# slatedb/slatedb

Measured on AMD Instinct MI355X. Metric: GiB/s device-resident SST block encode+bloom, 64 MiB sorted KV, 1/2/4/8 GPU, higher is better.
Workload: dtype u8

## Files before the change

slatedb_amd/csrc/sdb_api.cpp:

```cpp
#include <hip/hip_runtime.h>
#include <stdint.h>

#include <algorithm>
#include <mutex>
#include <vector>

#include "../../include/slatedb_amd.h"
#include "sdb_decode.h"
#include "sdb_bloom.h"
#include "sdb_compact.h"
#include "sdb_reads.h"

using namespace sdb;

namespace {

inline hipStream_t S(void *s) { return reinterpret_cast<hipStream_t>(s); }

uint16_t num_probes_for(uint32_t bpk) { return (uint16_t)((float)bpk * 0.69f); }

uint64_t filter_bytes_for(uint64_t n, uint32_t bpk) {
    uint32_t bits = (uint32_t)n * bpk;
    return bits / 8u + (bits % 8u != 0);
}
// ... 127 lines not shown
    s.nfacts = (uint32_t)((n + kFactsEntries - 1) / kFactsEntries);
    encode_ws_layout(n, s.wso);
    {
        uint32_t g = 16;
        while ((uint64_t)g * g < s.nchunks) g++;
        s.group = g;
    }
    *standalone_bloom = false;
    if (want_filter && prefix_filter(p)) {
        s.prefix_bloom = 1;
        s.bloom_len = 0;
        *standalone_bloom = true;
    } else if (want_filter && n) {
        const BloomPlan pl = bloom_plan(n, s.num_probes, fb, kChunk);
        if (bloom_plan_fits(pl)) {
            s.bloom_fused = 1;
            s.bpl = pl;
            s.slot_cap = bloom_slot_cap(pl);
        } else {
            *standalone_bloom = true;
        }
    }
    return s;
}

SstSet set_header(const sdb_sst_params *p) {
    SstSet P{};
    P.block_size = p->block_size;
    P.restart_interval = p->sst_version == 2 ? p->restart_interval : 1;
    P.version = p->sst_version;
    P.wal = p->sst_type == SDB_SST_WAL;
    const uint64_t look = (uint64_t)p->block_size / 12 + 2;
    P.seg_look = (uint32_t)(look < kSegLook ? look : kSegLook);
    return P;
}
}

extern "C" {

uint64_t sdb_encode_workspace_bytes(uint64_t n, const sdb_sst_params *params) {
    if (!params) return 0;
    return sst_ws_bytes(n, params) + 256;
}

uint64_t sdb_encode_ssts_workspace_bytes(uint32_t count, const sdb_kv_batch *batches, const sdb_sst_params *params) {
    if (!params || (count && !batches)) return 0;
    uint64_t t = 256;
    for (uint32_t i = 0; i < count; i++) t += sst_ws_bytes(batches[i].n, params);
    return t;
}

sdb_status sdb_encode_ssts(uint32_t count, const sdb_kv_batch *batches, const sdb_sst_params *p,
                           const sdb_sst_out *outs, void *workspace, uint64_t workspace_bytes, void *stream) {
    sdb_status st = check_params(p);
    if (st) return st;
    if (count && (!batches || !outs)) return SDB_INVALID_ARGUMENT;
    for (uint32_t i = 0; i < count; i++)
        if ((st = check_sst(&batches[i], p, &outs[i]))) return st;
    if (!device_ok()) return SDB_DEVICE_ERROR;
    if (!workspace || workspace_bytes < sdb_encode_ssts_workspace_bytes(count, batches, p)) return SDB_INVALID_ARGUMENT;
    hipStream_t s = S(stream);
    uint8_t *ws = ws_align(workspace);
    SstSet P = set_header(p);
    size_t bin_lds = 0, fill_lds = 0;
    auto flush = [&]() -> bool {
        const bool ok = launch_encode_set(P, bin_lds, fill_lds, s) == hipSuccess;
// ... 602 lines not shown
```

slatedb_amd/csrc/sdb_compact.hip:

```cpp
#include <hip/hip_runtime.h>

#include "sdb_compact.h"
#include "sdb_device.h"

namespace sdb {

namespace {

constexpr uint32_t kPfxThreads = 256;

SDB_DEV uint32_t run_of(const MergeArgs &a, uint64_t g) {
    uint32_t r = 0;
    for (uint32_t k = 1; k < a.nruns; k++) r += g >= a.r[k].base ? 1u : 0u;
    return r;
}

SDB_DEV RunDesc run_desc(const MergeArgs &a, uint32_t run) {
    RunDesc d = a.r[0];
    for (uint32_t k = 1; k < a.nruns; k++) {
        const RunDesc &c = a.r[k];
        const bool m = run == k;
        d.n = m ? c.n : d.n;
        d.base = m ? c.base : d.base;
        d.key_arena = m ? c.key_arena : d.key_arena;
// ... 728 lines not shown
                    e = n;
                    break;
                }
                acc += s_bb[o];
                if (acc > max_sst) {
                    if (j + 1 < n) cut[++ns] = j + 1;
                    acc = 0;
                    e = j + 1;
                    entry_pt = (e % kChunk) == 0;
                    continue;
                }
                entry_pt = j / kChunk != k;
                e = j;
            }
            s_stage = want;
        }
        __syncthreads();
        const uint64_t sv = s_stage;
        const uint64_t want = (uint64_t)(uint32_t)__builtin_amdgcn_readfirstlane((int)(uint32_t)sv) |
                              ((uint64_t)(uint32_t)__builtin_amdgcn_readfirstlane((int)(uint32_t)(sv >> 32)) << 32);
        if (want == kCutDone) break;
        if (want & kCutTables) {
            const uint64_t g = want & ~kCutTables, k0 = g * G, nk = k0 + G < K ? G : K - k0;
            for (uint32_t x = tid; x < nk * W; x += kCutThreads) {
                const uint32_t q = x / W, o = x - q * W;
                const uint64_t kk = k0 + q, ccs = kk * kChunk, cce = ccs + kChunk < n ? ccs + kChunk : n;
                s_cx[x] = ccs + o < cce ? a.tab_exit[kk * L + o] : 0xFFFFFFFFu;
                s_cb[x] = ccs + o < cce ? a.tab_bytes[kk * L + o] : 0;
            }
            gstaged = g;
        } else {
            const uint64_t cs = want * kChunk, ce = cs + kChunk < n ? cs + kChunk : n;
            for (uint64_t x = cs + tid; x < ce; x += kCutThreads) {
                s_next[x - cs] = a.next[x];
                s_bb[x - cs] = a.bbytes[x];
            }
            staged = want;
        }
        __syncthreads();
    }
    if (tid == 0) {
        if (n) cut[++ns] = n;
        *num = ns;
    }
}

__global__ void k_cut_offsets(const uint64_t *cut, const uint64_t *num, const uint64_t *key_off, const uint64_t *val_off,
                              uint64_t *out) {
    const uint64_t ns = *num;
    for (uint64_t i = (uint64_t)blockIdx.x * blockDim.x + threadIdx.x; i <= ns; i += (uint64_t)gridDim.x * blockDim.x) {
        const uint64_t c = cut[i];
        out[2 * i] = key_off[c];
        out[2 * i + 1] = val_off[c];
    }
}

__global__ void k_cx_blocks(CxInputs in, uint64_t *start, uint64_t *end) {
    const uint64_t nb = in.nblocks;
    for (uint64_t k = (uint64_t)blockIdx.x * blockDim.x + threadIdx.x; k < nb; k += (uint64_t)gridDim.x * blockDim.x) {
        uint32_t lo = 0, hi = in.n - 1;
        while (lo < hi) {
            const uint32_t mid = (lo + hi + 1) >> 1;
            if (in.first_block[mid] <= k) lo = mid;
            else hi = mid - 1;
        }
        const uint64_t j = k - in.first_block[lo], d = (uint64_t)(uintptr_t)in.data[lo] - in.base;
        start[k] = d + in.block_off[lo][j];
        end[k] = d + in.block_off[lo][j + 1];
// ... 156 lines not shown
```

slatedb_amd/csrc/sdb_encode.h:

```cpp
#pragma once
#include <hip/hip_runtime.h>
#include <stdint.h>

#include "../../include/slatedb_amd.h"
#include "sdb_workspace.h"

namespace sdb {

constexpr uint32_t kChunk = 2048;
constexpr uint32_t kResolveLds = 96 * 1024;
#ifndef SDB_EMIT_CRC_MFMA
#define SDB_EMIT_CRC_SLICE
#endif
#ifdef SDB_EMIT_CRC_SLICE
constexpr uint32_t kCrcLds = 36 * 1024;
#else
constexpr uint32_t kCrcLds = 56 * 1024;
#endif
constexpr uint32_t kImgCap = 4096 + 64;
constexpr uint32_t kStageCap = 4096;
constexpr uint32_t kStageGuard = 64;
constexpr uint32_t kKeyStageCap = 1024;
constexpr uint32_t kPieceRowMax = 4000, kPieceKeyMax = 960, kPieceValMax = 3968;
constexpr uint32_t kSegLook = 1024;
// ... 23 lines not shown
};
struct BloomSlots {
    uint32_t *count;
    uint32_t *slot;
    uint32_t cap;
};

struct BlockDesc {
    uint32_t s, e;
    uint64_t off;
    uint64_t vs, ve, ks, ke;
    uint32_t bb, route;
};
enum : uint32_t { kRouteImage = 0, kRouteWorkgroup = 1, kRoutePieces = 2 };
enum : uint32_t { kChunkHuge = 1, kChunkCarry = 2 };

struct EncodeArgs {
    const uint8_t *key_bytes;
    const uint64_t *key_off;
    const uint8_t *val_bytes;
    const uint64_t *val_off;
    const uint8_t *kind;
    const uint64_t *seq;
    const int64_t *create_ts;
    const int64_t *expire_ts;
    const uint8_t *ts_mask;
    uint64_t n;
    uint32_t block_size;
    uint32_t restart_interval;
    uint32_t version;
    uint32_t wal;
    uint32_t nchunks;
    uint32_t seg_look;
    uint32_t *lcp;
    uint32_t *szr, *sznr;
    uint32_t nfacts;
    uint32_t *row_scratch;
    uint32_t *next;
    uint32_t *bbytes;
    uint32_t *tab_exit;
    uint32_t *tab_cnt;
    uint64_t *tab_bytes;
    uint32_t *anchor_e;
    uint32_t *anchor_blk;
    uint64_t *anchor_byte;
    unsigned long long *err;
    uint32_t *wmax;
    uint32_t *slow_count;
    uint32_t *slow_list;
    uint32_t *big_count;
    uint32_t *big_list;
    BlockDesc *desc;
    uint64_t *stat_part;
    uint32_t *huge_part;
    uint32_t *wmax_part;
    unsigned long long *err_part;
    uint32_t *gtab_exit;
    uint32_t *gtab_cnt;
    uint64_t *gtab_bytes;
    uint32_t *pre_exit;
    uint32_t *pre_cnt;
    uint64_t *pre_bytes;
    uint32_t *anchor_arrived;
    uint32_t *mode;
    uint32_t group;
    uint32_t bloom_fused;
    BloomPlan bpl;
    BloomSlots bq;
    uint8_t *bloom_out;
    uint32_t *done;
    uint32_t nprep_wg;
    uint32_t seg_lds;
    uint8_t *out_data;
    uint64_t *out_block_off;
    uint32_t *out_block_first;
    uint32_t *out_index_key_len;
    uint16_t *out_block_stats;
    uint64_t data_cap, block_cap;
    sdb_sst_summary *summary;
    uint64_t bloom_len;
    uint32_t num_probes, filter_built;
    const uint64_t *bloom_len_dev;
};

#define SDB_ENCODE_WS(X)                                                                                      \
    X(lcp, uint32_t, n + 1)                                                                                   \
    X(szr, uint32_t, n + 1)                                                                                   \
    X(sznr, uint32_t, n + 1)                                                                                  \
    X(row_scratch, uint32_t, n + 1)                                                                           \
    X(next, uint32_t, n + 1)                                                                                  \
    X(bbytes, uint32_t, n + 1)                                                                                \
    X(tab_exit, uint32_t, nt)                                                                                 \
    X(tab_cnt, uint32_t, nt)                                                                                  \
    X(tab_bytes, uint64_t, nt)                                                                                \
    X(anchor_e, uint32_t, nc + 2)                                                                             \
    X(anchor_blk, uint32_t, nc + 2)                                                                           \
    X(anchor_byte, uint64_t, nc + 2)                                                                          \
    X(err, unsigned long long, 1)                                                                             \
    X(wmax, uint32_t, 1)                                                                                      \
    X(slow_count, uint32_t, 1)                                                                                \
    X(slow_list, uint32_t, n + 1)                                                                             \
    X(big_count, uint32_t, 1)                                                                                 \
    X(big_list, uint32_t, n + 1)                                                                              \
    X(desc, BlockDesc, n + 1)                                                                                 \
    X(stat_part, uint64_t, 5 * (nf + 1))                                                                      \
    X(huge_part, uint32_t, nf + 1)                                                                            \
    X(wmax_part, uint32_t, nc + 1)                                                                            \
    X(err_part, unsigned long long, nf + 1)                                                                   \
    X(done, uint32_t, 2)                                                                                      \
    X(gtab_exit, uint32_t, nt)                                                                                \
    X(gtab_cnt, uint32_t, nt)                                                                                 \
    X(gtab_bytes, uint64_t, nt)                                                                               \
    X(pre_exit, uint32_t, nt)                                                                                 \
    X(pre_cnt, uint32_t, nt)                                                                                  \
    X(pre_bytes, uint64_t, nt)                                                                                \
    X(anchor_arrived, uint32_t, 1)                                                                            \
    X(mode, uint32_t, 1)                                                                                      \
    X(bloom_len_dev, const uint64_t, 1)
enum WsField {
#define X(name, T, count) kWs_##name,
    SDB_ENCODE_WS(X)
#undef X
    kWsTail,
    kWsFields
// ... 26 lines not shown
                              const int32_t *qlens, uint64_t n, uint8_t *result, hipStream_t st);

constexpr uint32_t kMaxSsts = 8;
struct SstSlot {
    const uint8_t *key_bytes;
    const uint64_t *key_off;
    const uint8_t *val_bytes;
    const uint64_t *val_off;
    const uint8_t *kind;
    const uint64_t *seq;
    const int64_t *create_ts;
    const int64_t *expire_ts;
    const uint8_t *ts_mask;
    uint64_t n;
    uint8_t *out_data;
    uint64_t *out_block_off;
    uint32_t *out_block_first;
    uint32_t *out_index_key_len;
    uint16_t *out_block_stats;
    uint64_t data_cap, block_cap;
    sdb_sst_summary *summary;
    uint8_t *bloom_out;
    uint64_t bloom_len;
    uint8_t *ws;
    uint32_t num_probes, filter_built, bloom_fused;
    uint32_t prefix_bloom;
    uint32_t nchunks, nfacts, group, slot_cap;
    BloomPlan bpl;
    uint32_t wso[kWsFields];
};
struct SstSet {
    uint32_t count;
    uint32_t block_size, restart_interval, version, wal, seg_look;
    uint32_t max_facts, max_chunks, max_groups, max_tiles, max_slices, pad;
    SstSlot s[kMaxSsts];
};

__host__ __device__ inline EncodeArgs make_args(const SstSet &P, uint32_t i) {
    const SstSlot &s = P.s[i];
    EncodeArgs a{};
    a.key_bytes = s.key_bytes;
    a.key_off = s.key_off;
    a.val_bytes = s.val_bytes;
    a.val_off = s.val_off;
    a.kind = s.kind;
    a.seq = s.seq;
    a.create_ts = s.create_ts;
    a.expire_ts = s.expire_ts;
    a.ts_mask = s.ts_mask;
    a.n = s.n;
    a.block_size = P.block_size;
    a.restart_interval = P.restart_interval;
    a.version = P.version;
    a.wal = P.wal;
    a.nchunks = s.nchunks;
    a.seg_look = P.seg_look;
    a.nfacts = s.nfacts;
#define X(name, T, count) a.name = (T *)(s.ws + ((uint64_t)s.wso[kWs_##name] << 8));
    SDB_ENCODE_WS(X)
#undef X
    if (!s.prefix_bloom) a.bloom_len_dev = nullptr;
    a.group = s.group;
    a.bloom_fused = s.bloom_fused;
    a.bpl = s.bpl;
    a.bq.cap = s.slot_cap;
    bloom_slots_bind(a.bq, s.bpl, s.ws + ((uint64_t)s.wso[kWsTail] << 8));
    a.bloom_out = s.bloom_out;
    a.nprep_wg = s.nchunks;
    a.seg_lds = kSegLds;
    a.out_data = s.out_data;
    a.out_block_off = s.out_block_off;
    a.out_block_first = s.out_block_first;
    a.out_index_key_len = s.out_index_key_len;
    a.out_block_stats = s.out_block_stats;
    a.data_cap = s.data_cap;
    a.block_cap = s.block_cap;
    a.summary = s.summary;
    a.bloom_len = s.bloom_len;
    a.num_probes = s.num_probes;
    a.filter_built = s.filter_built;
    return a;
}

hipError_t launch_encode_set(const SstSet &P, size_t bin_lds, size_t fill_lds, hipStream_t st);
hipError_t launch_encode_empty(EncodeArgs a, hipStream_t st);
hipError_t launch_encode_prep(const SstSet &P, hipStream_t st);

enum Stage { kStBloom = 0, kStFacts, kStSeg, kStAnchor, kStBlocks, kStEmit, kStEmitBig, kStBloomFill, kNumStages };
void stage_mark(hipStream_t st, int stage, bool begin);
bool stage_timing_on();

BloomPlan bloom_plan(uint64_t n, uint32_t k, uint64_t bitmap_bytes, uint32_t tile_keys = 0);
uint64_t bloom_workspace_bytes(uint64_t n, uint32_t k, uint64_t bitmap_bytes);
hipError_t launch_bloom_build(const uint8_t *key_bytes, const uint64_t *key_off, uint64_t n,
                              uint32_t num_probes, uint8_t *bitmap, uint64_t bitmap_bytes, uint8_t *w,
                              hipStream_t st);
hipError_t launch_bloom_query(const uint8_t *bitmap, uint64_t bitmap_bytes, uint32_t num_probes,
                              const uint8_t *key_bytes, const uint64_t *key_off, uint64_t n,
                              uint8_t *result, hipStream_t st);

}
static_assert(sdb::kSegSpan % sdb::kSegThreads == 0 && sdb::kChunk % 64 == 0, "k_seg geometry");
static_assert(sdb::kEmitLds <= 160 * 1024, "k_emit LDS");
static_assert(sizeof(sdb::SstSet) <= 4096, "SstSet is passed as kernel arguments");
```

slatedb_amd/csrc/sdb_encode.hip:

```cpp
#include <stdlib.h>

#include <atomic>
#include <mutex>

#include "sdb_bloom.h"
#include "sdb_crc.h"
#include "sdb_crc_mfma.h"

namespace sdb {

#ifndef SDB_SEG_WAVES
#define SDB_SEG_WAVES 8
#endif
#ifdef SDB_PHASE_TIMING
__device__ uint64_t g_phase[1024][8];
#define PHASE_MARK(i)                                                              \
    do {                                                                           \
        __syncthreads();                                                           \
        if (threadIdx.x == 0 && blockIdx.x < 1024) g_phase[blockIdx.x][i] = __builtin_amdgcn_s_memtime(); \
    } while (0)
__device__ uint64_t g_wave_phase[8192][8];
__device__ uint64_t g_wave_rt[8192][4];
#define WAVE_T(var)                                     \
    uint64_t var = __builtin_amdgcn_s_memtime();        \
// ... 75 lines not shown
        else if (x1) lcp = 8 + (__builtin_ctzll(x1) >> 3);
        else if (nmin <= 16) lcp = nmin;
        else lcp = 16 + lcp_bytes(a.key_bytes + in.pko + 16, nmin - 16, a.key_bytes + in.ko0 + 16, nmin - 16);
        if (klen == 0) err = SDB_EMPTY_KEY;
        else if (!a.wal && plen > 0 && lcp == klen && klen < plen) err = SDB_INVALID_ARGUMENT;
    }
    if (!err && klen == 0) err = SDB_EMPTY_KEY;
    const uint32_t ts8 = 8u * (((m & SDB_TS_CREATE) != 0) + ((m & SDB_TS_EXPIRE) != 0));
    if (a.version == 2) {
        if (!err && (klen > 0xFFFFFFFFull || vlen > 0xFFFFFFFFull)) err = SDB_LIMIT_EXCEEDED;
        uint32_t kl = (uint32_t)klen, vl = (uint32_t)vlen, suf = kl - lcp;
        f.s_nr = varint_len(lcp) + varint_len(suf) + varint_len(vl) + suf + vl + 9 + ts8;
        f.s_r = 1 + varint_len(kl) + varint_len(vl) + kl + vl + 9 + ts8;
    } else {
        if (!err && (klen > 0xFFFF || vlen > 0xFFFFFFFFull)) err = SDB_LIMIT_EXCEEDED;
        f.s_r = (uint32_t)(4 + klen + 9 + ts8 + (kd == SDB_KIND_TOMBSTONE ? 0 : 4 + vlen));
        f.s_nr = f.s_r;
    }
    f.lcp = lcp;
    f.klen = klen;
    f.vlen = vlen;
    f.kind = kd;
    f.err = err;
    return f;
}

SDB_DEV EntryFacts entry_facts(const EncodeArgs &a, uint64_t i) {
    FactsIn in;
    facts_load_offsets(a, i, in);
    facts_load_keys(a, in);
    return facts_finish(a, i, in);
}

template <int CTRL>
SDB_DEV uint64_t dpp_or_own(uint64_t own, uint64_t v) {
    const uint32_t lo = (uint32_t)__builtin_amdgcn_update_dpp((int)(uint32_t)own, (int)(uint32_t)v, CTRL, 0xF, 0xF, false);
    const uint32_t hi =
        (uint32_t)__builtin_amdgcn_update_dpp((int)(uint32_t)(own >> 32), (int)(uint32_t)(v >> 32), CTRL, 0xF, 0xF, false);
    return (uint64_t)hi << 32 | lo;
}

__global__ __launch_bounds__(kFactsThreads, 8) void k_facts(SstSet P) {
    const EncodeArgs a = make_args(P, blockIdx.y);
    if (blockIdx.x >= a.nfacts) return;
    extern __shared__ __attribute__((aligned(16))) uint32_t blds[];
    __shared__ uint64_t s_part[kFactsThreads / 64][5];
    __shared__ unsigned long long s_err[kFactsThreads / 64];
    __shared__ uint32_t s_huge[kFactsThreads / 64];
    const uint32_t tid = threadIdx.x, lane = (uint32_t)lane_id();
    if (blockIdx.x == 0 && tid == 0) *a.anchor_arrived = 0;
    const uint64_t e0 = (uint64_t)blockIdx.x * kFactsEntries + tid;
    const uint64_t n = a.n;
    FactsIn in[kFactsPerT];
#pragma unroll
    for (uint32_t r = 0; r < kFactsPerT; r++) {
        const uint64_t e = e0 + r * kFactsThreads;
        FactsIn &f = in[r];
        f.ko0 = f.ko1 = f.vo0 = f.vo1 = f.pko = 0;
        f.kd = f.m = 0;
        if (e <= n) {
            f.ko0 = a.key_off[e];
            f.vo0 = a.val_off[e];
            if (e < n) {
                f.kd = a.kind ? a.kind[e] : 0;
                f.m = a.ts_mask ? a.ts_mask[e] : 0;
                if (lane == 63) {
// ... 38 lines not shown
        if (e < n && f.ko0 + 16 > ktot) {
            const uint64_t kl = f.ko1 - f.ko0;
            const uint32_t kn = (uint32_t)(kl < 16 ? kl : 16);
            f.ck0 = f.ck1 = 0;
            if (kn) f.ck0 = load8(a.key_bytes + f.ko0, kn < 8 ? kn : 8);
            if (kn > 8) f.ck1 = load8(a.key_bytes + f.ko0 + 8, kn - 8);
        }
        if (lane == 0 && e > 0 && e < n && f.pko + 16 > ktot) {
            const uint64_t pl = f.ko0 - f.pko;
            const uint32_t pn = (uint32_t)(pl < 16 ? pl : 16);
            f.pk0 = f.pk1 = 0;
            if (pn) f.pk0 = load8(a.key_bytes + f.pko, pn < 8 ? pn : 8);
            if (pn > 8) f.pk1 = load8(a.key_bytes + f.pko + 8, pn - 8);
        }
    }
    uint64_t rk = 0, rv = 0;
    uint32_t cv = 0, ct = 0, cm = 0;
    uint64_t err = ~0ull;
    bool huge = false;
    bool carry = false;
    uint32_t hh[kFactsPerT], dd[kFactsPerT];
#pragma unroll
    for (uint32_t r = 0; r < kFactsPerT; r++) {
        FactsIn &f = in[r];
        const uint64_t e = e0 + r * kFactsThreads;
        if (e == 0) f.pko = f.ko0;
        f.pko = dpp_or_own<kDppWaveShr1>(f.pko, f.ko0);
        f.pk0 = dpp_or_own<kDppWaveShr1>(f.pk0, f.ck0);
        f.pk1 = dpp_or_own<kDppWaveShr1>(f.pk1, f.ck1);
        hh[r] = dd[r] = 0;
        uint32_t kq = SDB_KIND_TOMBSTONE + 1;
        if (e < n) {
            const EntryFacts x = facts_finish(a, e, f);
            a.lcp[e] = x.lcp;
            a.szr[e] = x.s_r;
            a.sznr[e] = x.s_nr;
            if (a.bloom_fused) {
                const uint64_t kl = f.ko1 - f.ko0;
#ifdef SDB_EXP_FACTS_NOHASH
                const uint64_t h = (f.ck0 * 0x9E3779B97F4A7C15ull) ^ (f.ck1 + kl);
#else
                const uint64_t h = kl == 16 ? siphash13_16(f.ck0, f.ck1) : siphash13(a.key_bytes + f.ko0, kl);
#endif
                hh[r] = fastmod_u32((uint32_t)h, a.bpl.mmod, a.bpl.m);
                dd[r] = fastmod_u32((uint32_t)(h >> 32), a.bpl.mmod, a.bpl.m);
            }
            if (x.err) {
                const uint64_t ev = (e << 8) | (uint64_t)x.err;
                err = ev < err ? ev : err;
            }
            huge |= x.s_r > kPieceRowMax || x.klen > kPieceKeyMax || x.vlen > kPieceValMax;
            carry |= x.kind == SDB_KIND_TOMBSTONE && f.vo1 != f.vo0;
            rk += x.klen;
            rv += x.vlen;
            kq = x.kind;
        }
        cv += (uint32_t)__popcll(__ballot(kq == SDB_KIND_VALUE));
        ct += (uint32_t)__popcll(__ballot(kq == SDB_KIND_TOMBSTONE));
        cm += (uint32_t)__popcll(__ballot(kq == SDB_KIND_MERGE));
    }
    static_assert(64ull * kFactsPerT * (kPieceKeyMax > kPieceValMax ? kPieceKeyMax : kPieceValMax) < (1ull << 32),
                  "a wave's 32-bit sums");
    const bool wh = __ballot(huge) != 0, wc = __ballot(carry) != 0;
    if (wh) {
        rk = wave_sum(rk);
        rv = wave_sum(rv);
    } else {
        rk = wave_sum((uint32_t)rk);
        rv = wave_sum((uint32_t)rv);
// ... 34 lines not shown
#endif
    }
}

SDB_DEV uint32_t walk_size_v2(const EncodeArgs &a, uint64_t j, bool rs) {
    EntryFacts f = entry_facts(a, j);
    return rs ? f.s_r : f.s_nr;
}

SDB_DEV void seg_chunk(const EncodeArgs &a, uint8_t *smem, uint32_t k) {
    uint32_t *s_P = (uint32_t *)smem;
    uint32_t *s_R = s_P + kSegSpan + 4;
    uint32_t *s_bb = s_R + kSegSpan;
    uint16_t *s_nx = (uint16_t *)(s_bb + kChunk);
    __shared__ uint32_t s_len[kSegThreads / 64];
    const uint32_t tid = threadIdx.x, nt = blockDim.x;
    const uint64_t cs = (uint64_t)k * kChunk;
    const uint64_t ce = cs + kChunk < a.n ? cs + kChunk : a.n;
    const uint64_t se = ce + a.seg_look < a.n ? ce + a.seg_look : a.n;
    const uint32_t cn = (uint32_t)(ce - cs), sn = (uint32_t)(se - cs);
    const uint64_t bs = a.block_size;
    const uint32_t clampv = (uint32_t)(bs + 16);
    const bool v2 = a.version == 2 && bs <= (1u << 20);
    const uint32_t ri = a.restart_interval;
    PHASE_MARK(0);
    constexpr uint32_t kPerT = kSegSpan / kSegThreads;
    const uint32_t lane = (uint32_t)lane_id();
    uint32_t zr[kPerT], znr[kPerT];
#pragma unroll
    for (uint32_t u = 0; u < kPerT; u++) {
        const uint32_t x = tid + u * nt;
        zr[u] = znr[u] = 0;
        if (x < sn) {
            zr[u] = a.szr[cs + x];
            znr[u] = a.sznr[cs + x];
        }
    }
#pragma unroll
    for (uint32_t u = 0; u < kPerT; u++) {
        const uint32_t x = tid + u * nt;
        if (x >= sn) continue;
        if (v2) {
            const uint32_t cr = zr[u] < clampv ? zr[u] : clampv, cnr = znr[u] < clampv ? znr[u] : clampv;
            s_P[x] = cnr;
            s_R[x] = cr + 2 - cnr;
        }
    }
    __syncthreads();
    PHASE_MARK(1);
    if (v2) {
        __shared__ uint32_t s_wt[kPerT * (kSegThreads / 64) + 1];
        const uint32_t wv = tid >> 6;
        uint32_t v[kPerT], inc[kPerT];
#pragma unroll
        for (uint32_t u = 0; u < kPerT; u++) {
            const uint32_t x = tid + u * nt;
            v[u] = x < sn ? s_P[x] : 0;
            inc[u] = wave_incl_scan(v[u]);
            if (lane == 63) s_wt[u * (nt >> 6) + wv] = inc[u];
        }
        __syncthreads();
        if (tid < 64) {
            const uint32_t nw = kPerT * (nt >> 6);
            const uint32_t t = tid < nw ? s_wt[tid] : 0, it = wave_incl_scan(t);
            __builtin_amdgcn_wave_barrier();
            if (tid < nw) s_wt[tid] = it - t;
            if (tid == 63) s_P[sn] = it;
        }
// ... 3 lines not shown
            const uint32_t x = tid + u * nt;
            if (x < sn) s_P[x] = s_wt[u * (nt >> 6) + wv] + inc[u] - v[u];
        }
        PHASE_MARK(2);
    }
    __syncthreads();
    PHASE_MARK(3);
    uint32_t maxlen = 0;
    for (uint32_t x = tid; x < cn; x += nt) {
        const uint64_t b = cs + x;
        uint64_t j;
        uint64_t bytes;
        if (v2) {
            const uint32_t Pb = s_P[x];
            auto size_of = [&](uint32_t e) -> uint64_t {
                uint64_t sz = 2ull + (s_P[e] - Pb);
                for (uint32_t r = x; r < e; r += ri) sz += s_R[r];
                return sz;
            };
            uint32_t lo = x + 1;
            uint32_t e = lo;
            {
                const uint32_t w = (x + 64 < sn ? x + 64 : sn) - x;
                const uint32_t mean = (s_P[x + w] - Pb) / w + 1;
                uint32_t est = x + (uint32_t)(bs / mean);
                e = est < lo ? lo : (est > sn ? sn : est);
            }
            if (size_of(e) <= bs) {
                while (e < sn && size_of(e + 1) <= bs) e++;
            } else {
                while (e > lo && size_of(e) > bs) e--;
            }
            j = cs + e;
            if (e == lo) bytes = 2ull + a.szr[b] + 2;
            else bytes = size_of(e);
            if (e == sn && se < a.n) {
                uint64_t acc = bytes;
                uint32_t p = e - x, ph = p % ri;
                while (j < a.n) {
                    const bool rs = ph == 0;
                    const uint64_t add = (uint64_t)walk_size_v2(a, j, rs) + (rs ? 2 : 0);
                    if (acc + add > bs) break;
                    acc += add;
                    j++;
                    if (++ph == ri) ph = 0;
                }
                bytes = acc;
            }
        } else if (a.version == 2) {
            uint64_t acc = 2;
            j = b;
            uint32_t p = 0, ph = 0;
            while (j < a.n) {
                const bool rs = ph == 0;
                const uint64_t add = (uint64_t)walk_size_v2(a, j, rs) + (rs ? 2 : 0);
                if (p > 0 && acc + add > bs) break;
                acc += add;
                j++;
                p++;
                if (++ph == ri) ph = 0;
            }
            bytes = acc;
        } else {
            uint64_t acc = 2;
            j = b;
            uint32_t p = 0;
            const uint64_t fko = a.key_off[b];
            const uint32_t fkl = (uint32_t)(a.key_off[b + 1] - fko);
            while (j < a.n) {
                uint32_t prefix = 0;
                if (p > 0) {
                    uint64_t ko = a.key_off[j];
                    prefix = lcp_bytes(a.key_bytes + fko, fkl, a.key_bytes + ko, (uint32_t)(a.key_off[j + 1] - ko));
                }
                uint64_t sr = a.szr[j];
                uint64_t sz = sr - prefix;
                if (p > 0 && acc + sz > bs) break;
                acc += sz + 2;
                j++;
                p++;
            }
            bytes = acc;
        }
        const uint32_t bb = (uint32_t)(bytes + 4);
        a.next[b] = (uint32_t)j;
        a.bbytes[b] = bb;
        s_bb[x] = bb;
        const uint64_t rel = j - cs;
        s_nx[x] = (uint16_t)(rel < 0xFFFF ? rel : 0xFFFF);
        const uint32_t len = (uint32_t)(j - b);
        maxlen = len > maxlen ? len : maxlen;
    }
    maxlen = wave_max(maxlen);
    if (lane_id() == 0) s_len[tid >> 6] = maxlen;
    __syncthreads();
    if (tid == 0) {
        uint32_t m = 0;
        for (uint32_t q = 0; q < nt / 64; q++) m = s_len[q] > m ? s_len[q] : m;
        a.wmax_part[k] = m;
    }
    PHASE_MARK(4);
    __shared__ uint32_t s_wc;
    if (tid == 0) {
        uint32_t wc = a.seg_look;
        if (v2) {
            uint32_t lo = 0, hi = sn;
            while (lo < hi) {
                const uint32_t mid = (lo + hi + 1) >> 1;
                if ((uint64_t)(s_P[mid] - s_P[0]) + 2 <= bs) lo = mid;
                else hi = mid - 1;
            }
            wc = lo + 1 < wc ? lo + 1 : wc;
        }
        s_wc = wc;
    }
    __syncthreads();
    const uint32_t Wc = s_wc;
    uint32_t *j_nx = s_P;
    uint64_t *j_bb = (uint64_t *)(s_P + kChunk);
// ... 131 lines not shown
        a.done[1] = 0;
        *a.mode = W >= 1 && W <= a.seg_look ? 1u : 0u;
        sdb_sst_summary *sm = a.summary;
        auto total = [&](int f) {
            uint64_t t = 0;
            for (uint32_t q = 0; q < nt / 64; q++) t += s_stat[f][q];
            return t;
        };
        sm->raw_key_size = total(0);
        sm->raw_val_size = total(1);
        sm->num_puts = total(2);
        sm->num_deletes = total(3);
        sm->num_merges = total(4);
        sm->num_entries = a.n;
        sm->bloom_len = 0;
        sm->num_probes = 0;
        sm->filter_built = 0;
        sm->status = 0;
        sm->max_block_entries = 0;
        sm->first_error_entry = ~0ull;
    }
    return W;
}

SDB_DEV void chain_walk_serial(const EncodeArgs &a, uint64_t &blk, uint64_t &by) {
    uint64_t e = 0;
    blk = by = 0;
    for (uint32_t k = 0; k < a.nchunks; k++) {
        const uint64_t cs = (uint64_t)k * kChunk, ce = cs + kChunk < a.n ? cs + kChunk : a.n;
        a.anchor_e[k] = (uint32_t)e;
        a.anchor_blk[k] = (uint32_t)blk;
        a.anchor_byte[k] = by;
        while (e < ce) {
            by += a.bbytes[e];
            blk++;
            e = a.next[e];
        }
    }
}

SDB_DEV void chain_totals(const EncodeArgs &a, uint64_t blk, uint64_t by) {
    const uint32_t K = a.nchunks;
    a.anchor_e[K] = (uint32_t)a.n;
    a.anchor_blk[K] = (uint32_t)blk;
    a.anchor_byte[K] = by;
    a.summary->num_blocks = blk;
    a.summary->data_len = by;
    if (blk > a.block_cap || by > a.data_cap) report_error(a.err, 0, SDB_INVALID_ARGUMENT);
}

struct TabEntry {
    uint32_t x, c;
    uint64_t b;
};
SDB_DEV bool tab_in(const EncodeArgs &a, uint32_t k, uint32_t o) {
    const uint64_t cs = (uint64_t)k * kChunk, ce = cs + kChunk < a.n ? cs + kChunk : a.n;
    return cs + o < ce;
}
SDB_DEV TabEntry tab_clamp(const EncodeArgs &a, uint32_t k, uint32_t o, uint32_t W, uint32_t te, uint32_t tc,
                           uint64_t tb) {
    const uint64_t cs = (uint64_t)k * kChunk, ce = cs + kChunk < a.n ? cs + kChunk : a.n;
    const bool in = cs + o < ce;
    const uint64_t tx = te;
    return {in ? (tx >= ce && tx - ce < W ? (uint32_t)(tx - ce) : W - 1) : 0u, in ? tc : 0u, in ? tb : 0ull};
}
SDB_DEV TabEntry tab_load(const EncodeArgs &a, uint32_t k, uint32_t o, uint32_t W) {
    if (!tab_in(a, k, o)) return {0u, 0u, 0ull};
    const uint64_t t = (uint64_t)k * a.seg_look + o;
    return tab_clamp(a, k, o, W, a.tab_exit[t], a.tab_cnt[t], a.tab_bytes[t]);
// ... 390 lines not shown
        chain_totals(make_args(P, y), tb, ty);
    }
}

constexpr uint32_t kBlkThreads = 256;

__global__ __launch_bounds__(kBlkThreads) void k_blocks(SstSet P) {
    const EncodeArgs a = make_args(P, blockIdx.y);
    __shared__ uint16_t s_nx[kChunk];
    __shared__ uint32_t s_bb[kChunk];
    __shared__ uint16_t s_bs[kChunk];
    __shared__ uint64_t s_w[17];
    __shared__ uint32_t s_nbig, s_bigbase;
    __shared__ uint32_t s_big[kBlkThreads];
    const uint32_t k = blockIdx.x, K = a.nchunks;
    if (k >= K) return;
    if (*a.err != ~0ull) return;
    const uint32_t tid = threadIdx.x, nt = blockDim.x;
    const uint64_t cs = (uint64_t)k * kChunk, ce = cs + kChunk < a.n ? cs + kChunk : a.n;
    const uint32_t cn = (uint32_t)(ce - cs);
    const uint64_t e0 = a.anchor_e[k], byte0 = a.anchor_byte[k];
    const uint32_t blk0 = a.anchor_blk[k], nb = a.anchor_blk[k + 1] - blk0;
    if (blk0 + (uint64_t)nb > a.block_cap) {
        return;
    }
    if (k + 1 == K && tid == 0) {
        a.out_block_off[blk0 + nb] = a.anchor_byte[K];
        a.out_block_first[blk0 + nb] = (uint32_t)a.n;
    }
    if (!nb) return;
    {
        constexpr uint32_t kU = kChunk / kBlkThreads;
        uint32_t nx[kU], eb[kU];
#pragma unroll
        for (uint32_t u = 0; u < kU; u++) {
            const uint32_t x = u * nt + tid;
            nx[u] = x < cn ? a.next[cs + x] : 0;
            eb[u] = x < cn ? a.bbytes[cs + x] : 0;
        }
#pragma unroll
        for (uint32_t u = 0; u < kU; u++) {
            const uint32_t x = u * nt + tid;
            if (x < cn) {
                s_nx[x] = (uint16_t)(nx[u] >= ce ? cn : (uint32_t)(nx[u] - cs));
                s_bb[x] = eb[u];
            }
        }
    }
    if (tid == 0) s_nbig = 0;
    __syncthreads();
    if (tid == 0) {
        uint32_t x = (uint32_t)(e0 - cs);
        for (uint32_t t = 0; t < nb; t++) {
            s_bs[t] = (uint16_t)x;
            x = s_nx[x];
        }
    }
    __syncthreads();
    uint64_t carry = byte0;
    for (uint32_t b0 = 0; b0 < nb; b0 += nt) {
        const uint32_t t = b0 + tid;
        const bool v = t < nb;
        const uint32_t xs = v ? s_bs[t] : 0;
        const uint32_t bb = v ? s_bb[xs] : 0;
        uint64_t tot;
        const uint64_t off = carry + block_excl_scan_u64(bb, s_w, &tot);
        carry += tot;
        if (v) {
            const uint64_t s = cs + xs, e = t + 1 < nb ? cs + s_bs[t + 1] : a.next[s];
            const uint32_t blk = blk0 + t;
            a.out_block_off[blk] = off;
            a.out_block_first[blk] = (uint32_t)s;
            BlockDesc d;
            d.s = (uint32_t)s;
            d.e = (uint32_t)e;
            d.off = off;
            d.vs = a.val_off[s];
            d.ve = a.val_off[e];
            d.ks = a.key_off[s];
            d.ke = a.key_off[e];
            d.bb = bb;
            d.route = block_route(a, d);
            if (d.route == kRouteWorkgroup) a.slow_list[atomicAdd(a.slow_count, 1u)] = blk;
            if (d.route == kRoutePieces) s_big[atomicAdd(&s_nbig, 1u)] = blk;
            a.desc[blk] = d;
        }
        __syncthreads();
        const uint32_t nbig = s_nbig;
        if (nbig) {
            if (tid == 0) s_bigbase = atomicAdd(a.big_count, nbig);
            __syncthreads();
            for (uint32_t i = tid; i < nbig; i += nt) a.big_list[s_bigbase + i] = s_big[i];
            __syncthreads();
            if (tid == 0) s_nbig = 0;
            __syncthreads();
        }
    }
}

SDB_DEV void lds_put_bytes(lu8 *p, uint64_t w, uint32_t n) {
    for (uint32_t i = 0; i < n; i++) p[i] = (uint8_t)(w >> (8 * i));
}
// ... 757 lines not shown
            }
        }
    }
#ifdef SDB_PHASE_TIMING
    if (lane_id() == 0 && gw < 8192)
        for (int i = 0; i < 8; i++) g_wave_phase[gw][i] = ph[i];
    const uint64_t rt1 = __builtin_amdgcn_s_memrealtime(), mt1 = __builtin_amdgcn_s_memtime();
    if (lane_id() == 0 && gw < 8192) {
        g_wave_rt[gw][0] = rt0;
        g_wave_rt[gw][1] = rt1;
        g_wave_rt[gw][2] = mt0;
        g_wave_rt[gw][3] = mt1;
    }
#endif
    __syncthreads();
    if (threadIdx.x == 0) {
        __threadfence();
        if (atomicAdd(&make_args(P, 0).done[0], 1u) == gridDim.x - 1) {
            __threadfence();
            for (uint32_t i = 0; i < P.count; i++) finish_summary(make_args(P, i));
        }
    }
}

template <int V>
SDB_DEV void emit_slow_blocks(const EncodeArgs &a, uint8_t *scratch, const uint32_t (*s_crc)[256]) {
    uint8_t *s_win = scratch;
    uint64_t *s_size = (uint64_t *)(scratch + 8192);
    uint64_t *s_off = (uint64_t *)(scratch + 8192 + 8 * kEmitThreads);
    const uint32_t nslow = *a.slow_count;
    for (uint32_t it = blockIdx.x; it < nslow; it += gridDim.x) {
        const uint32_t blk = a.slow_list[it];
        const uint64_t b = a.out_block_first[blk];
        const uint64_t e = a.next[b];
        const uint64_t off = a.out_block_off[blk];
        const uint32_t ne = (uint32_t)(e - b);
        uint8_t *dst = a.out_data + off;
        const uint32_t ri = a.restart_interval;
        const uint64_t fko = a.key_off[b];
        const uint32_t fkl = (uint32_t)(a.key_off[b + 1] - fko);
        uint64_t D = 0;
        for (uint32_t i0 = 0; i0 < ne; i0 += blockDim.x) {
            uint32_t i = i0 + threadIdx.x;
            RowInfo r;
            uint64_t seq = 0;
            int64_t ets = 0, cts = 0;
            if (i < ne) {
                uint64_t j = b + i;
                uint64_t ko = a.key_off[j];
                uint32_t klen = (uint32_t)(a.key_off[j + 1] - ko);
                uint8_t kd = a.kind ? a.kind[j] : 0;
                uint8_t m = a.ts_mask ? a.ts_mask[j] : 0;
                uint32_t vlen = kd == SDB_KIND_TOMBSTONE ? 0 : (uint32_t)(a.val_off[j + 1] - a.val_off[j]);
                uint32_t shared;
                if (V == 2) shared = (i % ri == 0) ? 0 : a.lcp[j];
                else shared = (i == 0) ? 0 : lcp_bytes(a.key_bytes + fko, fkl, a.key_bytes + ko, klen);
                r.shared = shared;
                r.suf = klen - shared;
                r.vlen = vlen;
                r.key_src = ko + shared;
                r.val_src = a.val_off[j];
                r.flags = (uint8_t)((kd == SDB_KIND_MERGE ? SDB_FLAG_MERGE_OPERAND : 0) |
                                    (kd == SDB_KIND_TOMBSTONE ? SDB_FLAG_TOMBSTONE : 0) |
                                    ((m & SDB_TS_EXPIRE) ? SDB_FLAG_HAS_EXPIRE_TS : 0) |
                                    ((m & SDB_TS_CREATE) ? SDB_FLAG_HAS_CREATE_TS : 0));
                const uint32_t ts8 = 8u * (((m & SDB_TS_CREATE) != 0) + ((m & SDB_TS_EXPIRE) != 0));
                if (V == 2) r.size = varint_len(shared) + varint_len(r.suf) + varint_len(vlen) + r.suf + vlen + 9 + ts8;
                else r.size = 4 + r.suf + 9 + ts8 + (kd == SDB_KIND_TOMBSTONE ? 0 : 4 + vlen);
                seq = a.seq ? a.seq[j] : 0;
                ets = (m & SDB_TS_EXPIRE) ? a.expire_ts[j] : 0;
                cts = (m & SDB_TS_CREATE) ? a.create_ts[j] : 0;
                s_size[threadIdx.x] = r.size;
            } else {
                s_size[threadIdx.x] = 0;
            }
            __syncthreads();
            if (threadIdx.x == 0) {
                uint64_t c = D;
                for (uint32_t q = 0; q < blockDim.x; q++) {
                    s_off[q] = c;
                    c += s_size[q];
                }
            }
            __syncthreads();
            if (i < ne) {
                uint64_t ro = s_off[threadIdx.x];
                r.row_off = (uint32_t)ro;
                uint8_t *row = dst + ro;
                uint32_t h;
                write_row_small<V>(row, r, seq, ets, cts, &h);
                for (uint32_t q = 0; q < r.suf; q++) row[h + q] = a.key_bytes[r.key_src + q];
                uint32_t voff = (V == 2) ? h + r.suf : (r.size - r.vlen);
                for (uint32_t q = 0; q < r.vlen; q++) row[voff + q] = a.val_bytes[r.val_src + q];
                if (V == 2) {
                    if (i % ri == 0) {
                        if (ro > 0xFFFF) report_error(a.err, b + i, SDB_LIMIT_EXCEEDED);
                    }
                }
            }
            __syncthreads();
            if (i < ne) a.row_scratch[b + i] = (uint32_t)s_off[threadIdx.x];
            D = s_off[blockDim.x - 1] + s_size[blockDim.x - 1];
            __syncthreads();
        }
        __threadfence();
        __syncthreads();
        if (threadIdx.x == 0) {
            uint32_t pu = 0, de = 0, me = 0;
            for (uint64_t j = b; j < e; j++) {
                uint8_t kd = a.kind ? a.kind[j] : 0;
                pu += kd == SDB_KIND_VALUE;
                de += kd == SDB_KIND_TOMBSTONE;
                me += kd == SDB_KIND_MERGE;
            }
            a.out_block_stats[3 * (uint64_t)blk] = (uint16_t)pu;
            a.out_block_stats[3 * (uint64_t)blk + 1] = (uint16_t)de;
            a.out_block_stats[3 * (uint64_t)blk + 2] = (uint16_t)me;
            uint32_t ik = 0;
            if (b > 0 && !a.wal) {
                uint64_t fl = a.key_off[b + 1] - a.key_off[b];
                uint64_t pl = a.key_off[b] - a.key_off[b - 1];
                uint32_t lc = a.lcp[b];
                ik = (lc == pl && pl == fl) ? (uint32_t)fl : lc + 1;
            }
            a.out_index_key_len[blk] = ik;
        }
        uint32_t noffs = (V == 2) ? (ne + ri - 1) / ri : ne;
        for (uint32_t q = threadIdx.x; q < noffs; q += blockDim.x) {
            uint32_t ro = a.row_scratch[b + (V == 2 ? (uint64_t)q * ri : q)];
            dst[D + 2 * q] = (uint8_t)(ro >> 8);
            dst[D + 2 * q + 1] = (uint8_t)ro;
        }
        if (threadIdx.x == 0) {
            dst[D + 2 * noffs] = (uint8_t)(noffs >> 8);
            dst[D + 2 * noffs + 1] = (uint8_t)noffs;
        }
        __threadfence();
        __syncthreads();
        const uint64_t Lc = D + 2 * (uint64_t)noffs + 2;
        if (threadIdx.x < 64) {
            uint64_t nwin = (Lc + 4095) >> 12;
            uint64_t first = Lc - ((nwin - 1) << 12);
            uint32_t acc = 0;
            for (uint64_t w = 0; w < nwin; w++) {
                uint64_t wbeg = (w == 0) ? 0 : first + ((w - 1) << 12);
                uint32_t wlen = (uint32_t)((w == 0) ? first : 4096);
                for (uint32_t q = threadIdx.x; q < wlen; q += 64)
                    s_win[16 + q] = dst[wbeg + q] ^ (wbeg + q < 4 ? 0xFF : 0);
                wave_sync();
                uint32_t raw = wave_crc_raw_lds(s_win + 16, wlen, (const uint32_t(*)[256])s_crc, false);
                acc = (w == 0) ? raw : (gf_mul(c_shift.window, acc) ^ raw);
                wave_sync();
            }
            uint32_t crc = acc ^ 0xFFFFFFFFu;
            if (threadIdx.x == 0) {
// ... 207 lines not shown
```

Before: 1281.

## Narrow per-entry intermediates to 16-bit packed fields with escape fallbacks

Stores the per-entry LCP as uint16 with an escape value that triggers recomputation from key bytes. When version 2 is used and the block size fits in 16 bits, the two size arrays are packed into one word, and the next/bbytes chain into one 32-bit word, with overflow values spilled to the wide arrays. This cuts global memory traffic for workspace written and read across the prep, chain, anchor, cut and fill kernels. In exchange it adds branching, escape paths and possible extra loads for large entries.

```diff
diff --git a/slatedb_amd/csrc/sdb_api.cpp b/slatedb_amd/csrc/sdb_api.cpp
--- a/slatedb_amd/csrc/sdb_api.cpp
+++ b/slatedb_amd/csrc/sdb_api.cpp
@@ -183,6 +183,7 @@
     P.wal = p->sst_type == SDB_SST_WAL;
     const uint64_t look = (uint64_t)p->block_size / 12 + 2;
     P.seg_look = (uint32_t)(look < kSegLook ? look : kSegLook);
+    P.narrow = narrow_mode(P.version, P.block_size);
     return P;
 }
 }
diff --git a/slatedb_amd/csrc/sdb_compact.hip b/slatedb_amd/csrc/sdb_compact.hip
--- a/slatedb_amd/csrc/sdb_compact.hip
+++ b/slatedb_amd/csrc/sdb_compact.hip
@@ -784,8 +784,14 @@
         } else {
             const uint64_t cs = want * kChunk, ce = cs + kChunk < n ? cs + kChunk : n;
             for (uint64_t x = cs + tid; x < ce; x += kCutThreads) {
-                s_next[x - cs] = a.next[x];
-                s_bb[x - cs] = a.bbytes[x];
+                if (a.narrow) {
+                    const uint32_t w = a.chain[x];
+                    s_next[x - cs] = (uint32_t)chain_next_of(a, x, w);
+                    s_bb[x - cs] = chain_bytes_of(a, x, w);
+                } else {
+                    s_next[x - cs] = a.next[x];
+                    s_bb[x - cs] = a.bbytes[x];
+                }
             }
             staged = want;
         }
diff --git a/slatedb_amd/csrc/sdb_encode.h b/slatedb_amd/csrc/sdb_encode.h
--- a/slatedb_amd/csrc/sdb_encode.h
+++ b/slatedb_amd/csrc/sdb_encode.h
@@ -79,12 +79,15 @@
     uint32_t wal;
     uint32_t nchunks;
     uint32_t seg_look;
-    uint32_t *lcp;
+    uint32_t narrow;
+    uint16_t *lcp;
     uint32_t *szr, *sznr;
+    uint32_t *sz;
     uint32_t nfacts;
     uint32_t *row_scratch;
     uint32_t *next;
     uint32_t *bbytes;
+    uint32_t *chain;
     uint32_t *tab_exit;
     uint32_t *tab_cnt;
     uint64_t *tab_bytes;
@@ -131,12 +134,14 @@
 };
 
 #define SDB_ENCODE_WS(X)                                                                                      \
-    X(lcp, uint32_t, n + 1)                                                                                   \
+    X(lcp, uint16_t, n + 1)                                                                                   \
     X(szr, uint32_t, n + 1)                                                                                   \
     X(sznr, uint32_t, n + 1)                                                                                  \
+    X(sz, uint32_t, n + 1)                                                                                    \
     X(row_scratch, uint32_t, n + 1)                                                                           \
     X(next, uint32_t, n + 1)                                                                                  \
     X(bbytes, uint32_t, n + 1)                                                                                \
+    X(chain, uint32_t, n + 1)                                                                                 \
     X(tab_exit, uint32_t, nt)                                                                                 \
     X(tab_cnt, uint32_t, nt)                                                                                  \
     X(tab_bytes, uint64_t, nt)                                                                                \
@@ -229,7 +234,7 @@
 struct SstSet {
     uint32_t count;
     uint32_t block_size, restart_interval, version, wal, seg_look;
-    uint32_t max_facts, max_chunks, max_groups, max_tiles, max_slices, pad;
+    uint32_t max_facts, max_chunks, max_groups, max_tiles, max_slices, narrow;
     SstSlot s[kMaxSsts];
 };
 
@@ -252,6 +257,7 @@
     a.wal = P.wal;
     a.nchunks = s.nchunks;
     a.seg_look = P.seg_look;
+    a.narrow = P.narrow;
     a.nfacts = s.nfacts;
 #define X(name, T, count) a.name = (T *)(s.ws + ((uint64_t)s.wso[kWs_##name] << 8));
     SDB_ENCODE_WS(X)
@@ -279,6 +285,26 @@
     return a;
 }
 
+constexpr uint32_t kHalfEsc = 0xFFFF;
+inline bool narrow_mode(uint32_t version, uint32_t block_size) {
+    return version == 2 && (uint64_t)block_size + 16 < kHalfEsc;
+}
+__host__ __device__ inline uint32_t pack_sizes(uint32_t s_r, uint32_t s_nr, uint32_t clamp) {
+    return (s_nr < clamp ? s_nr : clamp) | (s_r < clamp ? s_r : clamp) << 16;
+}
+__host__ __device__ inline uint32_t pack_chain(uint64_t len, uint32_t bb) {
+    return (uint32_t)(len < kHalfEsc ? len : kHalfEsc) | (bb < kHalfEsc ? bb : kHalfEsc) << 16;
+}
+__device__ inline uint64_t chain_next_of(const EncodeArgs &a, uint64_t b, uint32_t w) {
+    return (w & 0xFFFF) != kHalfEsc ? b + (w & 0xFFFF) : a.next[b];
+}
+__device__ inline uint32_t chain_bytes_of(const EncodeArgs &a, uint64_t b, uint32_t w) {
+    return (w >> 16) != kHalfEsc ? w >> 16 : a.bbytes[b];
+}
+__device__ inline uint64_t chain_next(const EncodeArgs &a, uint64_t b) {
+    return a.narrow ? chain_next_of(a, b, a.chain[b]) : a.next[b];
+}
+
 hipError_t launch_encode_set(const SstSet &P, size_t bin_lds, size_t fill_lds, hipStream_t st);
 hipError_t launch_encode_empty(EncodeArgs a, hipStream_t st);
 hipError_t launch_encode_prep(const SstSet &P, hipStream_t st);
diff --git a/slatedb_amd/csrc/sdb_encode.hip b/slatedb_amd/csrc/sdb_encode.hip
--- a/slatedb_amd/csrc/sdb_encode.hip
+++ b/slatedb_amd/csrc/sdb_encode.hip
@@ -131,6 +131,14 @@
     return facts_finish(a, i, in);
 }
 
+SDB_DEV uint32_t lcp_at(const EncodeArgs &a, uint64_t j) {
+    const uint32_t l = a.lcp[j];
+    if (l != kHalfEsc) return l;
+    const uint64_t pk = a.key_off[j - 1], ck = a.key_off[j], ce = a.key_off[j + 1];
+    return kHalfEsc + lcp_bytes(a.key_bytes + pk + kHalfEsc, (uint32_t)(ck - pk) - kHalfEsc, a.key_bytes + ck + kHalfEsc,
+                                (uint32_t)(ce - ck) - kHalfEsc);
+}
+
 template <int CTRL>
 SDB_DEV uint64_t dpp_or_own(uint64_t own, uint64_t v) {
     const uint32_t lo = (uint32_t)__builtin_amdgcn_update_dpp((int)(uint32_t)own, (int)(uint32_t)v, CTRL, 0xF, 0xF, false);
@@ -235,9 +243,13 @@
         uint32_t kq = SDB_KIND_TOMBSTONE + 1;
         if (e < n) {
             const EntryFacts x = facts_finish(a, e, f);
-            a.lcp[e] = x.lcp;
-            a.szr[e] = x.s_r;
-            a.sznr[e] = x.s_nr;
+            a.lcp[e] = (uint16_t)(x.lcp < kHalfEsc ? x.lcp : kHalfEsc);
+            if (a.narrow) {
+                a.sz[e] = pack_sizes(x.s_r, x.s_nr, a.block_size + 16);
+            } else {
+                a.szr[e] = x.s_r;
+                a.sznr[e] = x.s_nr;
+            }
             if (a.bloom_fused) {
                 const uint64_t kl = f.ko1 - f.ko0;
 #ifdef SDB_EXP_FACTS_NOHASH
@@ -338,8 +350,19 @@
         const uint32_t x = tid + u * nt;
         zr[u] = znr[u] = 0;
         if (x < sn) {
-            zr[u] = a.szr[cs + x];
-            znr[u] = a.sznr[cs + x];
+            if (a.narrow) {
+                zr[u] = a.sz[cs + x];
+            } else {
+                zr[u] = a.szr[cs + x];
+                znr[u] = a.sznr[cs + x];
+            }
+        }
+    }
+    if (a.narrow) {
+#pragma unroll
+        for (uint32_t u = 0; u < kPerT; u++) {
+            znr[u] = zr[u] & 0xFFFF;
+            zr[u] >>= 16;
         }
     }
 #pragma unroll
@@ -409,8 +432,18 @@
                 while (e > lo && size_of(e) > bs) e--;
             }
             j = cs + e;
-            if (e == lo) bytes = 2ull + a.szr[b] + 2;
-            else bytes = size_of(e);
+            if (e == lo) {
+                uint32_t sr;
+                if (a.narrow) {
+                    sr = a.sz[b] >> 16;
+                    if (sr == clampv) sr = walk_size_v2(a, b, true);
+                } else {
+                    sr = a.szr[b];
+                }
+                bytes = 2ull + sr + 2;
+            } else {
+                bytes = size_of(e);
+            }
             if (e == sn && se < a.n) {
                 uint64_t acc = bytes;
                 uint32_t p = e - x, ph = p % ri;
@@ -460,8 +493,15 @@
             bytes = acc;
         }
         const uint32_t bb = (uint32_t)(bytes + 4);
-        a.next[b] = (uint32_t)j;
-        a.bbytes[b] = bb;
+        if (a.narrow) {
+            const uint32_t w = pack_chain(j - b, bb);
+            a.chain[b] = w;
+            if ((w & 0xFFFF) == kHalfEsc) a.next[b] = (uint32_t)j;
+            if ((w >> 16) == kHalfEsc) a.bbytes[b] = bb;
+        } else {
+            a.next[b] = (uint32_t)j;
+            a.bbytes[b] = bb;
+        }
         s_bb[x] = bb;
         const uint64_t rel = j - cs;
         s_nx[x] = (uint16_t)(rel < 0xFFFF ? rel : 0xFFFF);
@@ -659,9 +699,15 @@
         a.anchor_blk[k] = (uint32_t)blk;
         a.anchor_byte[k] = by;
         while (e < ce) {
-            by += a.bbytes[e];
+            if (a.narrow) {
+                const uint32_t w = a.chain[e];
+                by += chain_bytes_of(a, e, w);
+                e = chain_next_of(a, e, w);
+            } else {
+                by += a.bbytes[e];
+                e = a.next[e];
+            }
             blk++;
-            e = a.next[e];
         }
     }
 }
@@ -1118,11 +1164,26 @@
     {
         constexpr uint32_t kU = kChunk / kBlkThreads;
         uint32_t nx[kU], eb[kU];
-#pragma unroll
-        for (uint32_t u = 0; u < kU; u++) {
-            const uint32_t x = u * nt + tid;
-            nx[u] = x < cn ? a.next[cs + x] : 0;
-            eb[u] = x < cn ? a.bbytes[cs + x] : 0;
+        if (a.narrow) {
+#pragma unroll
+            for (uint32_t u = 0; u < kU; u++) {
+                const uint32_t x = u * nt + tid;
+                nx[u] = x < cn ? a.chain[cs + x] : 0;
+            }
+#pragma unroll
+            for (uint32_t u = 0; u < kU; u++) {
+                const uint32_t x = u * nt + tid;
+                const uint32_t w = nx[u];
+                nx[u] = x < cn ? (uint32_t)chain_next_of(a, cs + x, w) : 0;
+                eb[u] = x < cn ? chain_bytes_of(a, cs + x, w) : 0;
+            }
+        } else {
+#pragma unroll
+            for (uint32_t u = 0; u < kU; u++) {
+                const uint32_t x = u * nt + tid;
+                nx[u] = x < cn ? a.next[cs + x] : 0;
+                eb[u] = x < cn ? a.bbytes[cs + x] : 0;
+            }
         }
 #pragma unroll
         for (uint32_t u = 0; u < kU; u++) {
@@ -1153,7 +1214,7 @@
         const uint64_t off = carry + block_excl_scan_u64(bb, s_w, &tot);
         carry += tot;
         if (v) {
-            const uint64_t s = cs + xs, e = t + 1 < nb ? cs + s_bs[t + 1] : a.next[s];
+            const uint64_t s = cs + xs, e = t + 1 < nb ? cs + s_bs[t + 1] : chain_next(a, s);
             const uint32_t blk = blk0 + t;
             a.out_block_off[blk] = off;
             a.out_block_first[blk] = (uint32_t)s;
@@ -1977,7 +2038,7 @@
     for (uint32_t it = blockIdx.x; it < nslow; it += gridDim.x) {
         const uint32_t blk = a.slow_list[it];
         const uint64_t b = a.out_block_first[blk];
-        const uint64_t e = a.next[b];
+        const uint64_t e = chain_next(a, b);
         const uint64_t off = a.out_block_off[blk];
         const uint32_t ne = (uint32_t)(e - b);
         uint8_t *dst = a.out_data + off;
@@ -1998,7 +2059,7 @@
                 uint8_t m = a.ts_mask ? a.ts_mask[j] : 0;
                 uint32_t vlen = kd == SDB_KIND_TOMBSTONE ? 0 : (uint32_t)(a.val_off[j + 1] - a.val_off[j]);
                 uint32_t shared;
-                if (V == 2) shared = (i % ri == 0) ? 0 : a.lcp[j];
+                if (V == 2) shared = (i % ri == 0) ? 0 : lcp_at(a, j);
                 else shared = (i == 0) ? 0 : lcp_bytes(a.key_bytes + fko, fkl, a.key_bytes + ko, klen);
                 r.shared = shared;
                 r.suf = klen - shared;
@@ -2065,7 +2126,7 @@
             if (b > 0 && !a.wal) {
                 uint64_t fl = a.key_off[b + 1] - a.key_off[b];
                 uint64_t pl = a.key_off[b] - a.key_off[b - 1];
-                uint32_t lc = a.lcp[b];
+                uint32_t lc = lcp_at(a, b);
                 ik = (lc == pl && pl == fl) ? (uint32_t)fl : lc + 1;
             }
             a.out_index_key_len[blk] = ik;
```

New measurement: 1284, median of 6. Within noise of the previous version (+0.2%).
